# hermosayhl/CNN

Measured on AMD Instinct MI355X. Metric: images/sec (train step, 224x224x3), higher is better.
Workload: dtype f32; 1 GPU; reference AlexNet-style net (cpu/src/alexnet.cpp:10-33: 4x Conv3x3/s2 + ReLU, one MaxPool2x2, Linear 4608->3), full train step (fwd + softmax/CE + bwd + SGD), 224x224x3 fp32, BASELINE configs[1]; per_gpu_batch=256, global_batch=256, parallelism=dp1

## Files before the change

cnn_amd/csrc/common.h:

```cpp
#pragma once
#include <hip/hip_runtime.h>
#include <hip/hip_ext.h>

#include <atomic>
#include <cstdarg>
#include <cstdio>

#include "cnn_amd.h"

namespace cnn_amd {

char* error_buffer();
int fail(int code, const char* fmt, ...);

inline hipStream_t as_stream(void* s) { return reinterpret_cast<hipStream_t>(s); }

unsigned options_generation();
int num_cus();
struct DescMemo {
    struct Entry {
        cnn_conv2d_desc d;
        unsigned gen;
        int cus;
        bool used;
// ... 74 lines not shown
        if (e__ != hipSuccess)                                                                      \
            return ::cnn_amd::fail(CNN_AMD_E_HIP + (int)e__, "%s failed: %s", #expr, hipGetErrorString(e__)); \
    } while (0)

#define CNN_LAUNCH_CHECK() CNN_HIP_CHECK(hipGetLastError())

bool ktimer_active();
void ktimer_begin(hipStream_t s, const char* kernel, const char* fmt, ...);
void ktimer_end(hipStream_t s);

struct PublishState {
    hipEvent_t ev[2] = {nullptr, nullptr};
    int cur = 0, device = -1;
    bool armed = false;
    bool valid = false;
    bool stale = false;
    hipStream_t stream = nullptr;
};
PublishState& publish_state();
hipEvent_t publish_take(hipStream_t s);
int publish_after_launch(hipStream_t s);
void publish_mark_stale(hipStream_t s);
inline bool publish_busy() {
    const PublishState& p = publish_state();
    return p.armed || (p.valid && !p.stale);
}

template <typename... KArgs, typename... Args>
inline void launch_pub(void (*kern)(KArgs...), dim3 grid, dim3 block, unsigned shmem, hipStream_t s, Args&&... args) {
    hipEvent_t ev = publish_take(s);
    if (ev) hipExtLaunchKernelGGL(kern, grid, block, shmem, s, nullptr, ev, 0, static_cast<KArgs>(args)...);
    else hipLaunchKernelGGL(kern, grid, block, shmem, s, static_cast<KArgs>(args)...);
}

#define CNN_KLAUNCH(stream, kernel_name, expr, ...)                                         \
    do {                                                                                    \
        const bool t__ = ::cnn_amd::ktimer_active();                                        \
        if (t__) ::cnn_amd::ktimer_begin(stream, kernel_name, __VA_ARGS__);                 \
        expr;                                                                               \
        if (t__) ::cnn_amd::ktimer_end(stream);                                             \
        CNN_LAUNCH_CHECK();                                                                 \
        if (::cnn_amd::publish_busy())                                                      \
            if (int prc__ = ::cnn_amd::publish_after_launch(stream)) return prc__;          \
    } while (0)

#define CNN_REQUIRE(cond, ...)                                             \
    do {                                                                   \
        if (!(cond)) return ::cnn_amd::fail(CNN_AMD_E_BADARG, __VA_ARGS__); \
    } while (0)

__host__ __device__ inline int m16_filter_index(int j, int lane, int Ci, int slice) {
    return ((4 * (j / 9) + (lane >> 4)) * Ci + 16 * slice + (lane & 15)) * 9 + j % 9;
}

struct DeviceOnce {
    std::atomic<unsigned char> done[64];
    static int device() {
        int dev = 0;
        return (hipGetDevice(&dev) == hipSuccess && dev >= 0 && dev < 64) ? dev : -1;
    }
    bool needed() const {
        const int dev = device();
        return dev < 0 || done[dev].load(std::memory_order_acquire) == 0;
    }
    void mark() {
        const int dev = device();
        if (dev >= 0) done[dev].store(1, std::memory_order_release);
    }
};

__device__ __forceinline__ float sgd_one(float p, float g, float lr, float scale, bool scaled) {
#pragma clang fp contract(off)
    const float gs = scaled ? g * scale : g;
    const float step = lr * gs;
    return p - step;
}

template <bool kMomentum>
__device__ __forceinline__ float sgdm_one(float p, float g, float& v, float lr, float momentum, float wd, float scale, bool scaled,
                                          bool decay, bool nesterov) {
#pragma clang fp contract(off)
    const float gs = scaled ? g * scale : g;
    float d = gs;
    if (decay) {
        const float wp = wd * p;
        d = gs + wp;
    }
    float u = d;
    if (kMomentum) {
        const float mv = momentum * v;
        const float vn = mv + d;
        v = vn;
        if (nesterov) {
            const float mvn = momentum * vn;
            u = d + mvn;
        } else {
            u = vn;
        }
    }
    const float step = lr * u;
    return p - step;
}

constexpr int kWave = 64;
constexpr int kNumXCD = 8;

// ... 18 lines not shown
```

cnn_amd/csrc/conv_dgrad_rd.hip:

```cpp
#include <cstdlib>
#include <type_traits>

#include "common.h"

using namespace cnn_amd;

namespace cnn_amd {
bool igemm_preferred(const cnn_conv2d_desc* d, int mode);
}

namespace {

typedef float f32x16 __attribute__((ext_vector_type(16)));
struct __attribute__((packed, aligned(4))) f2u {
    float x, y;
};
struct __attribute__((packed, aligned(4))) f4u {
    float x, y, z, w;
};
typedef float v2f __attribute__((ext_vector_type(2)));
typedef float v4f __attribute__((ext_vector_type(4)));
struct Taps {
    v4f a, b;
    float c;
// ... 347 lines not shown
                const int g = g0 + ri, gp = g + NB - 1, rp = (ri + NB - 1) % NB;
                const bool wrap = gp >= G;
                const unsigned oo[3] = {wrap ? nxt.o[0] : cur.o[0], wrap ? nxt.o[1] : cur.o[1], wrap ? nxt.o[2] : cur.o[2]};
                load_group(ring[rp], wrap ? gp - G : gp, oo);
                RD_PIPE_FENCE(ring[ri].a[0][0][0]);
                (void)g;
#pragma unroll
                for (int u = 0; u < UC; ++u)
#pragma unroll
                    for (int kx = 0; kx < 3; ++kx) {
                        const f3u v = ring[ri].win[u][kx];
#pragma unroll
                        for (int ky = 0; ky < 3; ++ky) {
                            float d = cur.isz[ky] ? v.z : (cur.isy[ky] ? v.y : v.x);
                            d = cur.ok[kx][ky] ? d : 0.f;
#pragma unroll
                            for (int mt = 0; mt < MT; ++mt)
                                acc[mt] = __builtin_amdgcn_mfma_f32_32x32x2f32(ring[ri].a[u][mt][kx * 3 + ky], d, acc[mt], 0, 0, 0);
                        }
                    }
            }
        }
        if (cur.live) {
#pragma unroll
            for (int mt = 0; mt < MT; ++mt) {
                float m[16];
                if (p.relu_below) {
#pragma unroll
                    for (int r = 0; r < 16; ++r) {
                        const int rowl = mt * 32 + (r & 3) + 8 * (r >> 2) + 4 * kg;
                        m[r] = p.relu_below[(size_t)cur.xo + (size_t)(ci0 + rowl < p.Ci ? rowl : 0) * p.UV];
                    }
                }
#pragma unroll
                for (int r = 0; r < 16; ++r) {
                    const int rowl = mt * 32 + (r & 3) + 8 * (r >> 2) + 4 * kg;
                    if (ci0 + rowl >= p.Ci) continue;
                    float v = acc[mt][r];
                    if (p.relu_below) v = (m[r] <= 0.f) ? 0.f : v;
                    p.dx[(size_t)cur.xo + (size_t)rowl * p.UV] = v;
                }
            }
        }
        cur = nxt;
    }
}

#ifndef CNN_M16_DGRAD_NB
#define CNN_M16_DGRAD_NB 4
#endif
typedef float f32x4 __attribute__((ext_vector_type(4)));
constexpr unsigned kM16OOB = 0x7ffffffcu;

template <int CO, int NW, bool PREP, int KS, bool PD = false>
__global__ __launch_bounds__(NW * 64) void conv_dgrad_m16_s2_kernel(const DgRdParams p) {
    constexpr int C4 = CO / 4, NA = CO * 9 / 4;
    constexpr int NB = CNN_M16_DGRAD_NB;
    static_assert(C4 % NB == 0, "static ring indices");
    const int lane = threadIdx.x & 63;
    const int n = lane & 15, k = lane >> 4;
    const int slices = p.Ci >> 4;
    const int wid = xcd_swizzle(blockIdx.x, gridDim.x) * NW + (threadIdx.x >> 6);
    const int slice = wid % slices, half = KS > 1 ? (wid / slices) % KS : 0, wave_id = wid / (slices * KS);
    const int nwaves = p.tiles;
    const int groups = (p.pixels + 15) >> 4;
    if (wave_id >= nwaves || wave_id >= groups) return;
    float wa[NA];
    if constexpr (PREP) {
#pragma unroll
        for (int j = 0; j < NA; ++j) wa[j] = p.w[((half * slices + slice) * NA + j) * 64 + lane];
    } else {
#pragma unroll
        for (int j = 0; j < NA; ++j) wa[j] = p.w[half * CO * p.Ci * 9 + m16_filter_index(j, lane, p.Ci, slice)];
    }
    const int plane = p.Ho * p.Wo;
    const size_t hw = (size_t)p.H * p.W;
    const unsigned chs = (unsigned)hw * 4u;
    const bool odd = (p.W & 1) != 0;
    const __amdgpu_buffer_rsrc_t rsrc = __builtin_amdgcn_make_buffer_rsrc((void*)p.dy, 0, (int)((unsigned)p.B * CO * KS * plane * 4u), 0x00020000);
    const __amdgpu_buffer_rsrc_t xrs = __builtin_amdgcn_make_buffer_rsrc((void*)p.dx, 0, (int)((unsigned)p.B * p.Ci * (unsigned)hw * 4u), 0x00020000);
    const __amdgpu_buffer_rsrc_t mrs =
        __builtin_amdgcn_make_buffer_rsrc((void*)(p.relu_below ? p.relu_below : p.dx), 0, (int)((unsigned)p.B * p.Ci * (unsigned)hw * 4u), 0x00020000);
    struct Loc {
        unsigned o0, o1;
        bool ca, cb;
        unsigned x0, x1;
        bool w1;
        unsigned xq[2][2];
    };
    auto locate = [&](int g, Loc& L) {
        const int pix = g * 16 + n;
        const bool live = g < groups && pix < p.pixels;
        const int pp = live ? pix : 0;
        const int b = fdiv(pp, p.m_uv, p.UV);
        const int rem = pp - b * p.UV;
        const int u = fdiv(rem, p.m_v, p.V);
        const int v = rem - u * p.V;
        L.cb = v == 0;
        L.ca = !L.cb && v < p.Wo;
        const int cs = L.ca ? v - 1 : (L.cb ? 0 : p.Wo - 2);
        const unsigned base = (unsigned)((b * CO * KS + half * CO + k) * plane + u * p.Wo + cs) * 4u;
        L.o0 = (live && u < p.Ho) ? base : kM16OOB;
        L.o1 = (live && u >= 1) ? base - (unsigned)p.Wo * 4u : kM16OOB;
        if constexpr (PD) {
            const int y0 = 2 * u - 1, c0 = 2 * v - 1;
            const int xb = (int)((((size_t)b * p.Ci + 16 * slice + 4 * k) * hw) * 4u) + (y0 * p.W + c0) * 4;
#pragma unroll
            for (int ph = 0; ph < 2; ++ph)
#pragma unroll
                for (int pw = 0; pw < 2; ++pw) {
                    const bool ok = live && (unsigned)(y0 + ph) < (unsigned)p.H && (unsigned)(c0 + pw) < (unsigned)p.W;
                    L.xq[ph][pw] = ok ? (unsigned)(xb + (ph * p.W + pw) * 4) : kM16OOB;
                }
            L.x0 = L.x1 = kM16OOB;
            L.w1 = true;
        } else {
            const unsigned xb = (unsigned)(((size_t)b * p.Ci + 16 * slice + 4 * k) * hw + (size_t)(2 * u) * p.W + 2 * v) * 4u;
            L.x0 = live ? xb : kM16OOB;
            L.x1 = (live && 2 * u + 1 < p.H) ? xb + (unsigned)p.W * 4u : kM16OOB;
            L.w1 = 2 * v + 1 < p.W;
        }
    };
    auto load_g = [&](v2f (&buf)[2], int c4, const Loc& L) {
        const int so = c4 * 4 * plane * 4;
        buf[0] = __builtin_bit_cast(v2f, __builtin_amdgcn_raw_buffer_load_b64(rsrc, (int)L.o0, so, 0));
        buf[1] = __builtin_bit_cast(v2f, __builtin_amdgcn_raw_buffer_load_b64(rsrc, (int)L.o1, so, 0));
    };
    Loc cur, nxt;
    locate(wave_id, cur);
    v2f ring[NB][2];
#pragma unroll
    for (int i = 0; i < NB - 1; ++i) load_g(ring[i], i, cur);
    for (int g = wave_id; g < groups; g += nwaves) {
        locate(g + nwaves, nxt);
        v2f mk[4][2];
        if constexpr (PD) {
            if (p.relu_below && half == 0) {
#pragma unroll
                for (int r = 0; r < 4; ++r)
#pragma unroll
                    for (int ph = 0; ph < 2; ++ph) {
                        mk[r][ph].x = __builtin_bit_cast(float, __builtin_amdgcn_raw_buffer_load_b32(mrs, (int)cur.xq[ph][0], (int)(r * chs), 0));
                        mk[r][ph].y = __builtin_bit_cast(float, __builtin_amdgcn_raw_buffer_load_b32(mrs, (int)cur.xq[ph][1], (int)(r * chs), 0));
                    }
            }
        } else
        if (p.relu_below && half == 0) {
            const unsigned m0 = (cur.w1 || cur.x0 == kM16OOB) ? cur.x0 : cur.x0 - 4u, m1 = (cur.w1 || cur.x1 == kM16OOB) ? cur.x1 : cur.x1 - 4u;
#pragma unroll
            for (int r = 0; r < 4; ++r) {
                mk[r][0] = __builtin_bit_cast(v2f, __builtin_amdgcn_raw_buffer_load_b64(mrs, (int)m0, (int)(r * chs), 0));
                mk[r][1] = __builtin_bit_cast(v2f, __builtin_amdgcn_raw_buffer_load_b64(mrs, (int)m1, (int)(r * chs), 0));
            }
        }
        f32x4 acc[4];
#pragma unroll
        for (int c = 0; c < 4; ++c) acc[c] = f32x4{0.f, 0.f, 0.f, 0.f};
#pragma unroll
        for (int c4 = 0; c4 < C4; ++c4) {
            const int gn = c4 + NB - 1;
            load_g(ring[gn % NB], gn % C4, gn < C4 ? cur : nxt);
            RD_PIPE_FENCE(ring[c4 % NB][0]);
            const v2f r0 = ring[c4 % NB][0], r1 = ring[c4 % NB][1];
            const float d00 = cur.ca ? r0.y : (cur.cb ? r0.x : 0.f), d01 = cur.ca ? r0.x : (cur.cb ? 0.f : r0.y);
            const float d10 = cur.ca ? r1.y : (cur.cb ? r1.x : 0.f), d11 = cur.ca ? r1.x : (cur.cb ? 0.f : r1.y);
            const float* a = &wa[c4 * 9];
#define M16_STEP(ACC, A_, B_)                                              \
    ACC = __builtin_amdgcn_mfma_f32_16x16x4f32(A_, B_, ACC, 0, 0, 0); \
    __builtin_amdgcn_sched_barrier(0)
            M16_STEP(acc[1], a[1], d00);
            M16_STEP(acc[0], a[0], d00);
            M16_STEP(acc[2], a[3], d00);
            M16_STEP(acc[0], a[2], d01);
            M16_STEP(acc[3], a[4], d00);
            M16_STEP(acc[0], a[6], d10);
            M16_STEP(acc[1], a[7], d10);
            M16_STEP(acc[0], a[8], d11);
            M16_STEP(acc[2], a[5], d01);
#undef M16_STEP
        }
        if constexpr (KS > 1) {
            __shared__ float red[2][KS - 1][NW / KS][16][64];
            const int rb = ((g - wave_id) / nwaves) & 1;
            if (half > 0) {
#pragma unroll
                for (int c = 0; c < 4; ++c)
#pragma unroll
                    for (int r = 0; r < 4; ++r) red[rb][half - 1][slice][c * 4 + r][lane] = acc[c][r];
            }
            __syncthreads();
            if (half > 0) {
                cur = nxt;
                continue;
            }
#pragma unroll
            for (int h = 0; h < KS - 1; ++h)
#pragma unroll
                for (int c = 0; c < 4; ++c)
#pragma unroll
                    for (int r = 0; r < 4; ++r) acc[c][r] += red[rb][h][slice][c * 4 + r][lane];
        }
        if constexpr (PD) {
#pragma unroll
            for (int r = 0; r < 4; ++r)
#pragma unroll
                for (int ph = 0; ph < 2; ++ph) {
                    float v0 = acc[ph * 2][r], v1 = acc[ph * 2 + 1][r];
                    if (p.relu_below) {
                        v0 = (mk[r][ph].x <= 0.f) ? 0.f : v0;
                        v1 = (mk[r][ph].y <= 0.f) ? 0.f : v1;
                    }
                    __builtin_amdgcn_raw_buffer_store_b32(__builtin_bit_cast(unsigned, v0), xrs, (int)cur.xq[ph][0], (int)(r * chs), 0);
                    __builtin_amdgcn_raw_buffer_store_b32(__builtin_bit_cast(unsigned, v1), xrs, (int)cur.xq[ph][1], (int)(r * chs), 0);
                }
            cur = nxt;
            continue;
        }
        const unsigned pp0 = cur.w1 ? cur.x0 : kM16OOB, pp1 = cur.w1 ? cur.x1 : kM16OOB;
        const unsigned ss0 = cur.w1 ? kM16OOB : cur.x0, ss1 = cur.w1 ? kM16OOB : cur.x1;
#pragma unroll
        for (int r = 0; r < 4; ++r)
#pragma unroll
            for (int ph = 0; ph < 2; ++ph) {
                float v0 = acc[ph * 2][r], v1 = acc[ph * 2 + 1][r];
                if (p.relu_below) {
                    const float k0 = cur.w1 ? mk[r][ph].x : mk[r][ph].y;
                    v0 = (k0 <= 0.f) ? 0.f : v0;
                    v1 = (mk[r][ph].y <= 0.f) ? 0.f : v1;
                }
                typedef unsigned u2 __attribute__((ext_vector_type(2)));
                __builtin_amdgcn_raw_buffer_store_b64(__builtin_bit_cast(u2, v2f{v0, v1}), xrs, (int)(ph ? pp1 : pp0), (int)(r * chs), 0);
                if (odd) __builtin_amdgcn_raw_buffer_store_b32(__builtin_bit_cast(unsigned, v0), xrs, (int)(ph ? ss1 : ss0), (int)(r * chs), 0);
            }
        cur = nxt;
    }
}

inline unsigned magic_of(int d) { return (unsigned)((1ull << 32) / (unsigned)d) + 1u; }

struct DgRdPlan {
    DgRdParams p;
    int co, nw, cgroups, blocks_x, mt;
    bool m16;
    size_t lds, img_floats;
};

inline bool m16_wanted(const cnn_conv2d_desc* d) {
    if (d->s != 2 || !((d->Ci == 16 && d->Co == 32) || (d->Ci == 32 && d->Co == 64) || (d->Ci == 64 && d->Co == 128))) return false;
    if (d->pad != 0 && !(d->pad == 1 && d->Ci == 64 && d->Co == 128)) return false;
    if ((long long)d->B * d->Co * cnn_conv2d_out_dim(d->H, 3, 2, d->pad) * cnn_conv2d_out_dim(d->W, 3, 2, d->pad) >= (1ll << 29) ||
        (long long)d->B * d->Ci * d->H * d->W >= (1ll << 29))
        return false;
    const OptVal e = CNN_OPT_VAL("DGRAD_M16");
    if (e && atoi(e) == 0) return false;
    if (d->Ci >= 32 && e && atoi(e) == 1) return false;
    if (d->Ci == 64 && e && atoi(e) == 2) return false;
    return true;
}

bool make_plan(const cnn_conv2d_desc* d, DgRdPlan* pl) {
    if (d->k != 3 || (d->s != 2 && d->s != 1)) return false;
    if (d->pad != 0 && !(d->pad == 1 && d->s == 2 && m16_wanted(d))) return false;
    if (d->s == 1 && ((d->Co != 64 && d->Co != 128) || d->Ci % 32 != 0)) return false;
    if ((d->Co != 32 && d->Co != 64 && d->Co != 128) || d->Ci % 16 != 0) return false;
    pl->m16 = m16_wanted(d);
    if (d->Co == 32 && !pl->m16 && !((CNN_OPT_SET("DGRAD_RD32") && CNN_OPT_INT("DGRAD_RD32", 0) != 0))) return false;
    if (const OptVal e = CNN_OPT_VAL("DGRAD_RD"))
        if (atoi(e) == 0) return false;
    DgRdParams& p = pl->p;
    p.B = d->B; p.Ci = d->Ci; p.H = d->H; p.W = d->W;
    p.Ho = cnn_conv2d_out_dim(d->H, 3, d->s, d->pad);
    p.Wo = cnn_conv2d_out_dim(d->W, 3, d->s, d->pad);
    if (p.Ho < 1 || p.Wo < (d->s == 1 ? 3 : 2)) return false;
    if (d->s == 1) { p.U = d->H; p.V = d->W; }
    else { p.U = (d->H + 2 * d->pad + 1) / 2; p.V = (d->W + 2 * d->pad + 1) / 2; }
    p.UV = p.U * p.V;
    const long long pixels = (long long)d->B * p.UV;
    if (pixels >= (1ll << 30) || (long long)d->B * d->Ci * d->H * d->W >= (1ll << 31) || (long long)d->B * d->Co * p.Ho * p.Wo >= (1ll << 31))
        return false;
    p.pixels = (int)pixels;
    p.tiles = (int)((pixels + 31) / 32);
    p.m_uv = magic_of(p.UV);
    p.m_v = magic_of(p.V);
    p.dbg = CNN_MEASURE_INT("DGRAD_RD_DBG", 0);
    pl->co = d->Co;
    pl->mt = (d->s == 1 && d->Ci % 64 == 0) ? 2 : 1;
    if (const OptVal e = CNN_OPT_VAL("DGRAD_RD_MT")) pl->mt = (atoi(e) == 2 && d->s == 1 && d->Ci % 64 == 0) ? 2 : 1;
    pl->cgroups = (d->Ci + 32 * pl->mt - 1) / (32 * pl->mt);
// ... 18 lines not shown
    return true;
}

template <int CO, int NW>
int launch(const DgRdPlan& pl, hipStream_t s, const char* name, const cnn_conv2d_desc* d) {
    const int var = CNN_OPT_INT("DGRAD_RD_VAR", 0);
    auto kern = var == 3 ? conv_dgrad_rd_s2_kernel<CO, NW, 2, 2> : conv_dgrad_rd_s2_kernel<CO, NW, 2, 4>;
    const dim3 grid(pl.blocks_x, pl.cgroups);
    CNN_KLAUNCH(s, name, (kern<<<grid, NW * 64, pl.lds, s>>>(pl.p)), "B%d Ci%d %dx%d Co%d k%d s%d p%d", d->B, d->Ci, d->H, d->W,
                d->Co, d->k, d->s, d->pad);
    return CNN_AMD_OK;
}

inline int prepared_transposed() { return CNN_OPT_SET("DGRAD_RD_NOTR") ? 0 : 1; }

}

namespace cnn_amd {

bool dgrad_rd_supported(const cnn_conv2d_desc* d) {
    DgRdPlan pl;
    return make_plan(d, &pl);
}

size_t dgrad_rd_prepared_floats(const cnn_conv2d_desc* d) {
    DgRdPlan pl;
    return make_plan(d, &pl) ? pl.img_floats : 0;
}

int dgrad_rd_prepare_layout(const cnn_conv2d_desc* d, int* transposed) {
    DgRdPlan pl;
    if (!make_plan(d, &pl)) return 0;
    *transposed = pl.m16 ? 2 : prepared_transposed();
    return 1;
}

__global__ __launch_bounds__(256) void dgrad_rd_transpose_kernel(const float* __restrict__ w, float* __restrict__ img, int Co, int Ci) {
    const int total = Co * Ci * 9;
    for (int i = blockIdx.x * 256 + threadIdx.x; i < total; i += gridDim.x * 256) {
        const int ci = i % Ci, r = i / Ci, tap = r % 9, co = r / 9;
        img[i] = w[((size_t)co * Ci + ci) * 9 + tap];
    }
}

int dgrad_rd_backward_data(const cnn_conv2d_desc* d, const float* dy, const float* w, const float* img, const float* relu_below,
                           float* dx, void* ws, size_t ws_bytes, hipStream_t s) {
    DgRdPlan pl;
    if (!make_plan(d, &pl)) return fail(CNN_AMD_E_BADARG, "conv_dgrad_rd: geometry not covered");
    pl.p.dy = dy; pl.p.w = w ? w : img; pl.p.tr = w ? 0 : prepared_transposed(); pl.p.relu_below = relu_below; pl.p.dx = dx;
    if (pl.m16) {
        pl.p.tr = w ? 0 : 2;
        char nm[64];
        snprintf(nm, sizeof(nm), "conv_dgrad_rd<2,%d,m16>/dgrad%s", d->Co, relu_below ? "+relu" : "");
#define M16(CO_, PREP_, NW_, KS_)                                                                                                        \
    CNN_KLAUNCH(s, nm, (launch_pub(conv_dgrad_m16_s2_kernel<CO_, NW_, PREP_, KS_>, dim3(pl.blocks_x), dim3(NW_ * 64), 0, s, pl.p)), "B%d Ci%d %dx%d Co%d k%d s%d p%d", \
                d->B, d->Ci, d->H, d->W, d->Co, d->k, d->s, d->pad)
        if (d->Co == 32) { if (pl.p.tr == 2) M16(32, true, 4, 1); else M16(32, false, 4, 1); }
        else if (d->Co == 64) { if (pl.p.tr == 2) M16(64, true, 4, 1); else M16(64, false, 4, 1); }
        else if (d->pad == 1) {
#define M16P(PREP_)                                                                                                                        \
    CNN_KLAUNCH(s, nm, (launch_pub(conv_dgrad_m16_s2_kernel<64, 8, PREP_, 2, true>, dim3(pl.blocks_x), dim3(8 * 64), 0, s, pl.p)), "B%d Ci%d %dx%d Co%d k%d s%d p%d", \
                d->B, d->Ci, d->H, d->W, d->Co, d->k, d->s, d->pad)
            if (pl.p.tr == 2) M16P(true); else M16P(false);
#undef M16P
        }
        else { if (pl.p.tr == 2) M16(64, true, 8, 2); else M16(64, false, 8, 2); }
#undef M16
        return CNN_AMD_OK;
    }
    if (w && ws && ws_bytes >= pl.img_floats * sizeof(float) && prepared_transposed()) {
        const unsigned gx = (unsigned)((pl.img_floats + 255) / 256);
        CNN_KLAUNCH(s, "dgrad_rd_transpose", (dgrad_rd_transpose_kernel<<<gx > 512 ? 512 : gx, 256, 0, s>>>(w, (float*)ws, d->Co, d->Ci)),
                    "B%d Ci%d %dx%d Co%d k%d s%d p%d", d->B, d->Ci, d->H, d->W, d->Co, d->k, d->s, d->pad);
        pl.p.w = (const float*)ws;
        pl.p.tr = 1;
    }
    char name[64];
    snprintf(name, sizeof(name), "conv_dgrad_rd<2,%d>/dgrad%s", d->Co, relu_below ? "+relu" : "");
    if (d->s == 1) {
        const dim3 grid(pl.blocks_x, pl.cgroups);
        snprintf(name, sizeof(name), "conv_dgrad_rd<1,%d,%d>/dgrad%s", d->Co, pl.mt, relu_below ? "+relu" : "");
#define S1(CO_, MT_, UC_) CNN_KLAUNCH(s, name, (conv_dgrad_rd_s1_kernel<CO_, MT_, 4, UC_><<<grid, 256, 0, s>>>(pl.p)), "B%d Ci%d %dx%d Co%d k%d s%d p%d", \
                                      d->B, d->Ci, d->H, d->W, d->Co, d->k, d->s, d->pad)
        const int uc = CNN_OPT_INT("DGRAD_RD_UC", 1);
        if (d->Co == 64 && pl.mt == 2) S1(64, 2, 1);
        else if (d->Co == 64) { if (uc == 2) S1(64, 1, 2); else S1(64, 1, 1); }
        else if (pl.mt == 2) S1(128, 2, 1);
        else { if (uc == 2) S1(128, 1, 2); else S1(128, 1, 1); }
#undef S1
        return CNN_AMD_OK;
    }
    if (d->Ci == 16) {
        const dim3 grid(pl.blocks_x, pl.cgroups);
#define SH(CO_) CNN_KLAUNCH(s, name, (conv_dgrad_rd_s2_kernel<CO_, 4, 2, 4, true><<<grid, 256, 0, s>>>(pl.p)), "B%d Ci%d %dx%d Co%d k%d s%d p%d", \
                            d->B, d->Ci, d->H, d->W, d->Co, d->k, d->s, d->pad)
        if (d->Co == 32) SH(32); else if (d->Co == 64) SH(64); else SH(128);
#undef SH
        return CNN_AMD_OK;
    }
    if (d->Co == 32) return launch<32, 4>(pl, s, name, d);
    if (d->Co == 64) return launch<64, 4>(pl, s, name, d);
    return launch<128, 4>(pl, s, name, d);
}

}
```

cnn_amd/csrc/conv_fwd_rd.hip:

```cpp
#include <cstdlib>

#include "common.h"

using namespace cnn_amd;

namespace cnn_amd {
bool igemm_preferred(const cnn_conv2d_desc* d, int mode);
}

namespace {

typedef float f32x16 __attribute__((ext_vector_type(16)));
struct __attribute__((packed, aligned(4))) f3u {
    float x, y, z;
};

#define RD_PIPE_FENCE(reg) asm volatile("" : "+v"(reg) : : "memory")

struct FwdRdParams {
    const float* x;
    const float* w;
    const float* img;
    const float* bias;
    float* y;
// ... 116 lines not shown
    for (; tile < p.tiles; tile += tstep) {
        const bool more = tile + tstep < p.tiles;
        if (more) locate(tile + tstep, nxoff, nyoff, nlive);
        f32x16 acc[MT];
#pragma unroll
        for (int mt = 0; mt < MT; ++mt) acc[mt] = bias_r[mt];
#pragma unroll
        for (int g = 0; g < G; ++g) {
            const int bi = g & 1, ri = g % NB, gp = g + NB - 1;
            if (gp < G) load_group(xb[gp % NB], gp, xoff);
            else if (more) load_group(xb[gp % NB], gp - G, nxoff);
            load_filters(ab[bi ^ 1], g + 1 < G ? g + 1 : 0);
            RD_PIPE_FENCE(ab[bi][0]);
#pragma unroll
            for (int u = 0; u < UC; ++u)
#pragma unroll
                for (int kx = 0; kx < 3; ++kx) {
                    const f3u v = xb[ri][u * 3 + kx];
#pragma unroll
                    for (int ky = 0; ky < 3; ++ky) {
                        const float bv = ky == 0 ? v.x : ky == 1 ? v.y : v.z;
#pragma unroll
                        for (int mt = 0; mt < MT; ++mt)
                            acc[mt] = __builtin_amdgcn_mfma_f32_32x32x2f32(ab[bi][((u * 3 + kx) * 3 + ky) * MT + mt], bv, acc[mt], 0, 0, 0);
                    }
                }
        }
        const long long dbg_t2 = p.dbg ? clock64() : 0;
        if (live) {
#pragma unroll
            for (int mt = 0; mt < MT; ++mt)
#pragma unroll
                for (int r = 0; r < 16; ++r) {
                    const int rowl = mt * 32 + (r & 3) + 8 * (r >> 2);
                    if (co0 + rowl + 4 * kg < p.Co) {
                        const size_t o = (size_t)yoff + (size_t)rowl * p.HoWo;
                        const float v = acc[mt][r];
                        if (p.y) p.y[o] = v;
                        if (p.y2) p.y2[o] = v >= 0.f ? v : 0.f;
                    }
                }
        }
        if (p.dbg && threadIdx.x == 0 && (blockIdx.x | blockIdx.y) == 0)
            printf("conv_fwd_rd wg 0: upload %lld, to end of MFMAs %lld, stores issued %lld cycles after start\n", dbg_t1 - dbg_t0,
                   dbg_t2 - dbg_t0, clock64() - dbg_t0);
        xoff = nxoff;
        yoff = nyoff;
        live = nlive;
    }
}

typedef float f32x4 __attribute__((ext_vector_type(4)));

__host__ __device__ inline int m16f_filter_index(int i, int Ci) {
    const int NA = Ci * 9 / 4;
    const int lane = i & 63, j = (i >> 6) % NA, slice = (i >> 6) / NA;
    return ((16 * slice + (lane & 15)) * Ci + 4 * (j / 9) + (lane >> 4)) * 9 + j % 9;
}

template <int S, int CI, int NW, bool PREP, int NB, int MS>
__global__ __launch_bounds__(NW * 64) void conv_fwd_m16_kernel(const FwdRdParams p) {
    constexpr int C4 = CI / 4, NA = C4 * 9;
    static_assert(C4 % NB == 0, "static ring indices");
    const int lane = threadIdx.x & 63;
    const int n = lane & 15, k = lane >> 4;
    const int slices = (p.Co >> 4) / MS, parts = p.tiles;
    const int wid = xcd_swizzle(blockIdx.x, gridDim.x) * NW + (threadIdx.x >> 6);
    const int slice = wid % slices, part = wid / slices;
    const int groups = (p.pixels + 15) >> 4;
    if (part >= parts || part >= groups) return;
    float wa[MS][NA], bs[MS][4];
#pragma unroll
    for (int m = 0; m < MS; ++m) {
        const int sl = slice * MS + m;
        if constexpr (PREP) {
#pragma unroll
            for (int j = 0; j < NA; ++j) wa[m][j] = p.img[(sl * NA + j) * 64 + lane];
        } else {
#pragma unroll
            for (int j = 0; j < NA; ++j) wa[m][j] = p.w[((16 * sl + n) * CI + 4 * (j / 9) + k) * 9 + j % 9];
        }
#pragma unroll
        for (int r = 0; r < 4; ++r) bs[m][r] = p.bias[16 * sl + 4 * k + r];
    }
    const long long dbg_t0 = p.dbg ? clock64() : 0;
    long long dbg_t1 = 0;
    int dbg_groups = 0;
    const unsigned plane = (unsigned)(p.H * p.W);
    auto locate = [&](int g, unsigned& xoff, unsigned& yoff, bool& live) {
        const int pi = g * 16 + n;
        live = g < groups && pi < p.pixels;
        const int pic = live ? pi : p.pixels - 1;
        const int b = fdiv(pic, p.m_howo, p.HoWo), rem = pic - b * p.HoWo;
        const int pr = fdiv(rem, p.m_wo, p.Wo), q = rem - pr * p.Wo;
        xoff = (unsigned)((b * CI + k) * (int)plane + (S * pr) * p.W + S * q);
        yoff = (unsigned)((b * p.Co + 16 * MS * slice + 4 * k) * p.HoWo + rem);
    };
    auto load_g = [&](f3u (&buf)[3], int c4, unsigned xoff) {
#pragma unroll
        for (int kx = 0; kx < 3; ++kx) {
            const float* base = p.x + ((size_t)(c4 * 4) * plane + (size_t)kx * p.W);
            buf[kx] = *(const f3u*)(base + xoff);
        }
    };
    unsigned xoff, yoff, nxoff, nyoff;
    bool live, nlive;
    locate(part, xoff, yoff, live);
    f3u xb[NB][3];
#pragma unroll
    for (int i = 0; i < NB - 1; ++i) load_g(xb[i], i, xoff);
    for (int g = part; g < groups; g += parts) {
        locate(g + parts, nxoff, nyoff, nlive);
        constexpr int NACC = 2;
        f32x4 acc[MS][NACC];
#pragma unroll
        for (int m = 0; m < MS; ++m) {
            acc[m][0] = f32x4{bs[m][0], bs[m][1], bs[m][2], bs[m][3]};
#pragma unroll
            for (int a = 1; a < NACC; ++a) acc[m][a] = f32x4{0.f, 0.f, 0.f, 0.f};
        }
#pragma unroll
        for (int c4 = 0; c4 < C4; ++c4) {
            const int gn = c4 + NB - 1;
            load_g(xb[gn % NB], gn % C4, gn < C4 ? xoff : nxoff);
            RD_PIPE_FENCE(xb[c4 % NB][0].x);
#pragma unroll
            for (int i = 0; i < 9; ++i) {
                const f3u v = xb[c4 % NB][i / 3];
                const float bv = i % 3 == 0 ? v.x : i % 3 == 1 ? v.y : v.z;
                const int a = (c4 * 9 + i) % NACC;
#pragma unroll
                for (int m = 0; m < MS; ++m) {
                    acc[m][a] = __builtin_amdgcn_mfma_f32_16x16x4f32(wa[m][c4 * 9 + i], bv, acc[m][a], 0, 0, 0);
                    __builtin_amdgcn_sched_barrier(0);
                }
            }
        }
        if (live) {
#pragma unroll
            for (int mr = 0; mr < MS * 4; ++mr) {
                const int m = mr >> 2, r = mr & 3;
                const float v = acc[m][0][r] + acc[m][1][r];
                const size_t o = (size_t)yoff + (size_t)(16 * m + r) * p.HoWo;
                if (p.y) p.y[o] = v;
                if (p.y2) p.y2[o] = v >= 0.f ? v : 0.f;
            }
        }
        xoff = nxoff;
        yoff = nyoff;
        live = nlive;
        if (p.dbg) {
            if (!dbg_groups) dbg_t1 = clock64();
            ++dbg_groups;
        }
    }
    if (p.dbg && threadIdx.x == 0 && blockIdx.x == 0)
        printf("conv_fwd_m16 wg 0: first group done %lld, all %d groups %lld cycles after the filter loads were issued\n", dbg_t1 - dbg_t0, dbg_groups,
               clock64() - dbg_t0);
}

inline unsigned magic_of(int d) { return (unsigned)((1ull << 32) / (unsigned)d) + 1u; }

struct FwdRdPlan {
    FwdRdParams p;
    int s, ci, mt, nw, cgroups, blocks_x;
    bool m16;
    int m16_blocks, m16_parts, m16_ms;
    size_t lds, img_floats;
};

bool make_plan(const cnn_conv2d_desc* d, FwdRdPlan* pl) {
    if (d->k != 3 || d->pad != 0 || (d->s != 1 && d->s != 2)) return false;
    if (d->Ci != 16 && d->Ci != 32 && d->Ci != 64) return false;
    if (const OptVal e = CNN_OPT_VAL("FWD_RD"))
        if (atoi(e) == 0) return false;
    FwdRdParams& p = pl->p;
    p.B = d->B; p.H = d->H; p.W = d->W; p.Co = d->Co;
    p.Ho = cnn_conv2d_out_dim(d->H, 3, d->s, 0);
    p.Wo = cnn_conv2d_out_dim(d->W, 3, d->s, 0);
    if (p.Ho <= 0 || p.Wo <= 0) return false;
    p.HoWo = p.Ho * p.Wo;
    const long long pixels = (long long)d->B * p.HoWo;
    if (pixels >= (1ll << 30) || (long long)d->B * d->Ci * d->H * d->W >= (1ll << 31) || pixels * d->Co >= (1ll << 31)) return false;
    p.pixels = (int)pixels;
    p.tiles = (int)((pixels + 31) / 32);
    p.m_howo = magic_of(p.HoWo);
    p.m_wo = magic_of(p.Wo);
    p.dbg = CNN_MEASURE_INT("FWD_RD_DBG", 0);
    pl->s = d->s;
    pl->ci = d->Ci;
    const int mtiles = (d->Co + 31) / 32;
    int mt = mtiles >= 2 && (long long)p.tiles * ((mtiles + 1) / 2) >= 4 * 4 * num_cus() ? 2 : 1;
    if ((size_t)(mt * 32 + 1) * d->Ci * 9 * 4 > 96 * 1024) mt = 1;
    if (const OptVal e = CNN_OPT_VAL("FWD_RD_MT")) mt = atoi(e) == 2 && mtiles >= 2 ? 2 : 1;
    pl->mt = mt;
    pl->cgroups = (mtiles + mt - 1) / mt;
    pl->img_floats = ((size_t)(mt * 32 + 1) * d->Ci * 9 + mt * 32 + 3) / 4 * 4;
    pl->lds = pl->img_floats * sizeof(float);
    pl->nw = pl->lds > 80 * 1024 ? 8 : 4;
    const int env = CNN_OPT_INT("FWD_RD_BLOCKS", 0);
    long long bx = (env > 0 ? env : (pl->nw == 8 ? num_cus() : 2 * num_cus())) / pl->cgroups;
    const long long need = (p.tiles + pl->nw - 1) / pl->nw;
    if (bx > need) bx = need;
    if (bx < 1) bx = 1;
    pl->blocks_x = (int)bx;
    const bool m16_ok = d->Co % 16 == 0 && (long long)d->B * d->Ci * d->H * d->W < (1ll << 29);
    const bool thin = d->Ci == 16 && d->Co % 32 == 0 && !((CNN_OPT_SET("FWD_M16_THIN") && CNN_OPT_INT("FWD_M16_THIN", 0) == 0));
    pl->m16 = m16_ok && ((long long)p.tiles * mtiles < 4 * 4 * num_cus() || thin);
    if (const OptVal e = CNN_OPT_VAL("FWD_M16")) pl->m16 = m16_ok && atoi(e) != 0;
    if (pl->m16) {
        pl->m16_ms = (d->Co % 32 == 0 && d->Ci <= 32 && !((CNN_OPT_SET("FWD_M16_MS") && CNN_OPT_INT("FWD_M16_MS", 0) == 1))) ? 2 : 1;
        const int slices = d->Co / 16 / pl->m16_ms, groups = (int)((pixels + 15) / 16);
        int per_simd = CNN_OPT_INT("FWD_M16_WAVES", (d->Ci == 16 ? 2 : 1));
        if (per_simd < 1 || per_simd > 8) per_simd = 1;
        int parts = per_simd * 4 * num_cus() / slices;
        if (parts < 1) parts = 1;
        if (parts > groups) parts = groups;
        pl->m16_parts = parts;
        pl->m16_blocks = (parts * slices + 3) / 4;
    }
    if (!pl->m16 && cnn_amd::igemm_preferred(d, 0)) return false;
    return true;
}

template <int S, int CI, int MT, int NW>
int launch(const FwdRdPlan& pl, hipStream_t s, const char* name, const cnn_conv2d_desc* d) {
    auto kern = conv_fwd_rd_kernel<S, CI, MT, NW, 2>;
    static DeviceOnce attr_once;
    if (attr_once.needed()) {
        CNN_HIP_CHECK(hipFuncSetAttribute((const void*)kern, hipFuncAttributeMaxDynamicSharedMemorySize, 160 * 1024));
        attr_once.mark();
    }
    const dim3 grid(pl.blocks_x, pl.cgroups);
    CNN_KLAUNCH(s, name, (kern<<<grid, NW * 64, pl.lds, s>>>(pl.p)), "B%d Ci%d %dx%d Co%d k%d s%d p%d", d->B, d->Ci, d->H, d->W,
                d->Co, d->k, d->s, d->pad);
    return CNN_AMD_OK;
}

struct FwdRdPrepJob {
    int kind;
    const float* w;
    const float* bias;
    float* img;
    int Co, Ci, cb, img_floats, cgroups, tr;
};
struct FwdRdPrepBatch {
    FwdRdPrepJob job[12];
};

__global__ __launch_bounds__(256) void fwd_rd_prepare_kernel(const FwdRdPrepBatch pb) {
    const FwdRdPrepJob j = pb.job[blockIdx.y];
    if (j.kind == 2) {
        const int total = j.Co * j.Ci * 9;
        for (int i = blockIdx.x * 256 + threadIdx.x; i < total; i += gridDim.x * 256) j.img[i] = j.w[m16f_filter_index(i, j.Ci)];
        return;
    }
    if (j.kind == 1) {
        const int total = j.Co * j.Ci * 9;
        for (int i = blockIdx.x * 256 + threadIdx.x; i < total; i += gridDim.x * 256) {
            if (j.tr == 2) {
                const int coh = j.Co > 64 ? j.Co / 2 : j.Co, na = coh * 9 / 4, slices = j.Ci / 16;
                const int jj = (i >> 6) % na, blk = (i >> 6) / na, slice = blk % slices, half = blk / slices;
                j.img[i] = j.w[half * coh * j.Ci * 9 + m16_filter_index(jj, i & 63, j.Ci, slice)];
            } else if (j.tr) {
                const int ci = i % j.Ci, r = i / j.Ci, tap = r % 9, co = r / 9;
                j.img[i] = j.w[((size_t)co * j.Ci + ci) * 9 + tap];
            } else {
                j.img[i] = j.w[i];
            }
        }
        return;
    }
    const int K = j.Ci * 9, cbp = j.cb + 1, total = j.cgroups * j.img_floats;
    for (int i = blockIdx.x * 256 + threadIdx.x; i < total; i += gridDim.x * 256) {
        const int g = i / j.img_floats, o = i - g * j.img_floats;
        float v = 0.f;
        if (o < K * cbp) {
            const int k = o / cbp, c = o - k * cbp, co = g * j.cb + c;
            if (c < j.cb && co < j.Co) v = j.w[(size_t)co * K + k];
        } else if (o < K * cbp + j.cb) {
            const int co = g * j.cb + (o - K * cbp);
            if (co < j.Co) v = j.bias[co];
        }
        j.img[i] = v;
    }
}

}

namespace cnn_amd {

bool fwd_rd_supported(const cnn_conv2d_desc* d) {
    FwdRdPlan pl;
    return make_plan(d, &pl);
}
bool fwd_rd_small(const cnn_conv2d_desc* d) {
    FwdRdPlan pl;
    return make_plan(d, &pl) && pl.m16;
}

size_t fwd_rd_prepared_floats(const cnn_conv2d_desc* d) {
    FwdRdPlan pl;
    if (!make_plan(d, &pl)) return 0;
    const size_t a = pl.img_floats * pl.cgroups, b = (size_t)d->Co * d->Ci * 9;
    return a > b ? a : b;
}

int dgrad_rd_prepare_layout(const cnn_conv2d_desc* d, int* transposed);

int rd_prepare_batch(int n, const cnn_conv2d_desc* descs, const float* const* w, const float* const* bias, void* const* fwd,
                     void* const* dgrad, hipStream_t s, unsigned* fdone, unsigned* ddone) {
    FwdRdPrepBatch pb;
    int jobs = 0;
    size_t most = 0;
    for (int i = 0; i < n && i < 6; ++i) {
        FwdRdPlan pl;
        if (fwd && fwd[i] && !(*fdone >> i & 1u) && make_plan(&descs[i], &pl)) {
            CNN_REQUIRE(w[i] && bias[i], "cnn_conv2d_prepare_filters: filters / bias of layer %d are null", i);
            FwdRdPrepJob& j = pb.job[jobs++];
            j.kind = pl.m16 ? 2 : 0; j.w = w[i]; j.bias = bias[i]; j.img = (float*)fwd[i];
            j.Co = descs[i].Co; j.Ci = descs[i].Ci; j.cb = pl.mt * 32; j.img_floats = (int)pl.img_floats; j.cgroups = pl.cgroups; j.tr = 0;
            if (pl.img_floats * pl.cgroups > most) most = pl.img_floats * pl.cgroups;
            *fdone |= 1u << i;
        }
        int tr = 0;
        if (dgrad && dgrad[i] && !(*ddone >> i & 1u) && dgrad_rd_prepare_layout(&descs[i], &tr)) {
            CNN_REQUIRE(w[i] != nullptr, "cnn_conv2d_prepare_filters: filters of layer %d are null", i);
            FwdRdPrepJob& j = pb.job[jobs++];
            j.kind = 1; j.w = w[i]; j.bias = nullptr; j.img = (float*)dgrad[i];
            j.Co = descs[i].Co; j.Ci = descs[i].Ci; j.cb = 0; j.img_floats = 0; j.cgroups = 0; j.tr = tr;
            const size_t nf = (size_t)descs[i].Co * descs[i].Ci * 9;
            if (nf > most) most = nf;
            *ddone |= 1u << i;
        }
    }
    if (jobs) {
        unsigned gx = (unsigned)((most + 255) / 256);
        if (gx > 512) gx = 512;
        CNN_KLAUNCH(s, "rd_prepare", (fwd_rd_prepare_kernel<<<dim3(gx, jobs), 256, 0, s>>>(pb)), "jobs=%d", jobs);
    }
    return CNN_AMD_OK;
}

int fwd_rd_forward(const cnn_conv2d_desc* d, const float* x, const float* w, const float* img, const float* bias, float* y,
                   float* y_relu, hipStream_t s) {
    FwdRdPlan pl;
    if (!make_plan(d, &pl)) return fail(CNN_AMD_E_BADARG, "conv_fwd_rd: geometry not covered");
    pl.p.x = x; pl.p.w = w; pl.p.img = w ? nullptr : img; pl.p.bias = bias; pl.p.y = y; pl.p.y2 = y_relu;
    char name[64];
    if (pl.m16) {
        pl.p.tiles = pl.m16_parts;
        snprintf(name, sizeof(name), "conv_fwd_rd<%d,%d,m16>/fwd%s", d->s, d->Ci, y_relu ? "+relu" : "");
#define M16K(S_, CI_, PREP_, MS_)                                                                                                            \
    CNN_KLAUNCH(s, name, (launch_pub(conv_fwd_m16_kernel<S_, CI_, 4, PREP_, 4, MS_>, dim3(pl.m16_blocks), dim3(256), 0, s, pl.p)), "B%d Ci%d %dx%d Co%d k%d s%d p%d", \
                d->B, d->Ci, d->H, d->W, d->Co, d->k, d->s, d->pad)
#define M16(S_, CI_)                                                          \
    do {                                                                      \
        if (pl.m16_ms == 2 && CI_ <= 32) {                                    \
            if (pl.p.img) M16K(S_, (CI_ <= 32 ? CI_ : 32), true, 2);         \
            else M16K(S_, (CI_ <= 32 ? CI_ : 32), false, 2);                 \
        } else {                                                              \
            if (pl.p.img) M16K(S_, CI_, true, 1);                             \
            else M16K(S_, CI_, false, 1);                                     \
        }                                                                     \
    } while (0)
        if (d->s == 2) { if (d->Ci == 16) M16(2, 16); else if (d->Ci == 32) M16(2, 32); else M16(2, 64); }
        else { if (d->Ci == 16) M16(1, 16); else if (d->Ci == 32) M16(1, 32); else M16(1, 64); }
#undef M16K
#undef M16
        return CNN_AMD_OK;
    }
    snprintf(name, sizeof(name), "conv_fwd_rd<%d,%d,%d>/fwd%s", d->s, d->Ci, pl.mt, y_relu ? "+relu" : "");
#define GO(S_, CI_)                                                                                  \
    do {                                                                                             \
        if (pl.mt == 2 && pl.nw == 8) return launch<S_, CI_, 2, 8>(pl, s, name, d);                  \
        if (pl.mt == 2) return launch<S_, CI_, 2, 4>(pl, s, name, d);                                \
        if (pl.nw == 8) return launch<S_, CI_, 1, 8>(pl, s, name, d);                                \
        return launch<S_, CI_, 1, 4>(pl, s, name, d);                                                \
    } while (0)
    if (d->s == 2) {
        if (d->Ci == 16) GO(2, 16); else if (d->Ci == 32) GO(2, 32); else GO(2, 64);
    } else {
        if (d->Ci == 16) GO(1, 16); else if (d->Ci == 32) GO(1, 32); else GO(1, 64);
    }
#undef GO
    return CNN_AMD_OK;
}

}
```

Measured before the change: 606,700 images/sec.

## Stream m16 conv filter loads into first group and vectorize prepacked filter image

The m16 forward and dgrad conv kernels used to load all filter registers before starting the input pipeline. Now they load only the first ring slices up front and fetch the rest per channel chunk inside the first group's loop, so filter fetch overlaps the input and gradient loads. The prepared filter image is re-laid out so each lane reads a 16-byte float4 quad, with a scalar fallback when the image is not 16-byte aligned. The rework adds template variants and a debug timing path, and may raise register pressure or change the instruction schedule.

```diff
diff --git a/cnn_amd/csrc/common.h b/cnn_amd/csrc/common.h
--- a/cnn_amd/csrc/common.h
+++ b/cnn_amd/csrc/common.h
@@ -150,6 +150,30 @@
 __host__ __device__ inline int m16_filter_index(int j, int lane, int Ci, int slice) {
     return ((4 * (j / 9) + (lane >> 4)) * Ci + 16 * slice + (lane & 15)) * 9 + j % 9;
 }
+__host__ __device__ inline int m16f_filter_index(int j, int lane, int Ci, int slice) {
+    return ((16 * slice + (lane & 15)) * Ci + 4 * (j / 9) + (lane >> 4)) * 9 + j % 9;
+}
+
+struct M16Slot {
+    int bank, j, lane;
+};
+__host__ __device__ inline M16Slot m16_image_slot(int i, int NA) {
+    const int q = i >> 2, na4 = NA / 4;
+    return M16Slot{(q >> 6) / na4, 4 * ((q >> 6) % na4) + (i & 3), q & 63};
+}
+#define M16_INLINE __attribute__((always_inline))
+#define M16_MEM_FENCE() asm volatile("" ::: "memory")
+template <bool V16>
+__device__ __forceinline__ void m16_load_quad(const float* img, int bank, int na4, int j4, int lane, float* r) {
+    const float* q = img + (size_t)__builtin_amdgcn_readfirstlane((bank * na4 + j4) * 256);
+    if constexpr (V16) {
+        const float4 v = ((const float4*)q)[lane];
+        r[0] = v.x; r[1] = v.y; r[2] = v.z; r[3] = v.w;
+    } else {
+#pragma unroll
+        for (int e = 0; e < 4; ++e) r[e] = q[4 * lane + e];
+    }
+}
 
 struct DeviceOnce {
     std::atomic<unsigned char> done[64];
diff --git a/cnn_amd/csrc/conv_dgrad_rd.hip b/cnn_amd/csrc/conv_dgrad_rd.hip
--- a/cnn_amd/csrc/conv_dgrad_rd.hip
+++ b/cnn_amd/csrc/conv_dgrad_rd.hip
@@ -423,9 +423,10 @@
 typedef float f32x4 __attribute__((ext_vector_type(4)));
 constexpr unsigned kM16OOB = 0x7ffffffcu;
 
-template <int CO, int NW, bool PREP, int KS, bool PD = false>
+template <int CO, int NW, int FL, int KS, bool PD = false>
 __global__ __launch_bounds__(NW * 64) void conv_dgrad_m16_s2_kernel(const DgRdParams p) {
     constexpr int C4 = CO / 4, NA = CO * 9 / 4;
+    static_assert(NA % 4 == 0, "whole 16-byte elements");
     constexpr int NB = CNN_M16_DGRAD_NB;
     static_assert(C4 % NB == 0, "static ring indices");
     const int lane = threadIdx.x & 63;
@@ -436,14 +437,6 @@
     const int nwaves = p.tiles;
     const int groups = (p.pixels + 15) >> 4;
     if (wave_id >= nwaves || wave_id >= groups) return;
-    float wa[NA];
-    if constexpr (PREP) {
-#pragma unroll
-        for (int j = 0; j < NA; ++j) wa[j] = p.w[((half * slices + slice) * NA + j) * 64 + lane];
-    } else {
-#pragma unroll
-        for (int j = 0; j < NA; ++j) wa[j] = p.w[half * CO * p.Ci * 9 + m16_filter_index(j, lane, p.Ci, slice)];
-    }
     const int plane = p.Ho * p.Wo;
     const size_t hw = (size_t)p.H * p.W;
     const unsigned chs = (unsigned)hw * 4u;
@@ -492,7 +485,7 @@
             L.w1 = 2 * v + 1 < p.W;
         }
     };
-    auto load_g = [&](v2f (&buf)[2], int c4, const Loc& L) {
+    auto load_g = [&](v2f (&buf)[2], int c4, const Loc& L) M16_INLINE {
         const int so = c4 * 4 * plane * 4;
         buf[0] = __builtin_bit_cast(v2f, __builtin_amdgcn_raw_buffer_load_b64(rsrc, (int)L.o0, so, 0));
         buf[1] = __builtin_bit_cast(v2f, __builtin_amdgcn_raw_buffer_load_b64(rsrc, (int)L.o1, so, 0));
@@ -502,9 +495,8 @@
     v2f ring[NB][2];
 #pragma unroll
     for (int i = 0; i < NB - 1; ++i) load_g(ring[i], i, cur);
-    for (int g = wave_id; g < groups; g += nwaves) {
-        locate(g + nwaves, nxt);
-        v2f mk[4][2];
+    v2f mk[4][2];
+    auto load_mask = [&]() M16_INLINE {
         if constexpr (PD) {
             if (p.relu_below && half == 0) {
 #pragma unroll
@@ -524,6 +516,29 @@
                 mk[r][1] = __builtin_bit_cast(v2f, __builtin_amdgcn_raw_buffer_load_b64(mrs, (int)m1, (int)(r * chs), 0));
             }
         }
+    };
+    load_mask();
+    M16_MEM_FENCE();
+    float wa[NA];
+    auto load_filters = [&](int c0, int c1) M16_INLINE {
+        if constexpr (FL != 0) {
+#pragma unroll
+            for (int j4 = 0; j4 < NA / 4; ++j4)
+                if (4 * j4 >= 9 * c0 && 4 * j4 < 9 * c1) m16_load_quad<FL == 2>(p.w, half * slices + slice, NA / 4, j4, lane, &wa[4 * j4]);
+        } else {
+#pragma unroll
+            for (int j = 0; j < NA; ++j)
+                if (j >= 9 * c0 && j < 9 * c1) wa[j] = p.w[half * CO * p.Ci * 9 + m16_filter_index(j, lane, p.Ci, slice)];
+        }
+    };
+    load_filters(0, NB - 1);
+    M16_MEM_FENCE();
+    const long long dbg_t0 = p.dbg ? clock64() : 0;
+    long long dbg_t1 = 0;
+    int dbg_groups = 0;
+    auto group = [&](int g, bool first) M16_INLINE {
+        locate(g + nwaves, nxt);
+        if (!first) load_mask();
         f32x4 acc[4];
 #pragma unroll
         for (int c = 0; c < 4; ++c) acc[c] = f32x4{0.f, 0.f, 0.f, 0.f};
@@ -531,6 +546,7 @@
         for (int c4 = 0; c4 < C4; ++c4) {
             const int gn = c4 + NB - 1;
             load_g(ring[gn % NB], gn % C4, gn < C4 ? cur : nxt);
+            if (first && gn < C4) load_filters(gn, gn + 1);
             RD_PIPE_FENCE(ring[c4 % NB][0]);
             const v2f r0 = ring[c4 % NB][0], r1 = ring[c4 % NB][1];
             const float d00 = cur.ca ? r0.y : (cur.cb ? r0.x : 0.f), d01 = cur.ca ? r0.x : (cur.cb ? 0.f : r0.y);
@@ -562,7 +578,7 @@
             __syncthreads();
             if (half > 0) {
                 cur = nxt;
-                continue;
+                return;
             }
 #pragma unroll
             for (int h = 0; h < KS - 1; ++h)
@@ -585,7 +601,11 @@
                     __builtin_amdgcn_raw_buffer_store_b32(__builtin_bit_cast(unsigned, v1), xrs, (int)cur.xq[ph][1], (int)(r * chs), 0);
                 }
             cur = nxt;
-            continue;
+            if (p.dbg) {
+                if (!dbg_groups) dbg_t1 = clock64();
+                ++dbg_groups;
+            }
+            return;
         }
         const unsigned pp0 = cur.w1 ? cur.x0 : kM16OOB, pp1 = cur.w1 ? cur.x1 : kM16OOB;
         const unsigned ss0 = cur.w1 ? kM16OOB : cur.x0, ss1 = cur.w1 ? kM16OOB : cur.x1;
@@ -604,7 +624,16 @@
                 if (odd) __builtin_amdgcn_raw_buffer_store_b32(__builtin_bit_cast(unsigned, v0), xrs, (int)(ph ? ss1 : ss0), (int)(r * chs), 0);
             }
         cur = nxt;
-    }
+        if (p.dbg) {
+            if (!dbg_groups) dbg_t1 = clock64();
+            ++dbg_groups;
+        }
+    };
+    group(wave_id, true);
+    for (int g = wave_id + nwaves; g < groups; g += nwaves) group(g, false);
+    if (p.dbg && threadIdx.x == 0 && blockIdx.x == 0)
+        printf("conv_dgrad_m16 wg 0: first group done %lld, all %d groups %lld cycles after the filter loads were issued\n", dbg_t1 - dbg_t0,
+               dbg_groups, clock64() - dbg_t0);
 }
 
 inline unsigned magic_of(int d) { return (unsigned)((1ull << 32) / (unsigned)d) + 1u; }
@@ -729,19 +758,20 @@
         pl.p.tr = w ? 0 : 2;
         char nm[64];
         snprintf(nm, sizeof(nm), "conv_dgrad_rd<2,%d,m16>/dgrad%s", d->Co, relu_below ? "+relu" : "");
-#define M16(CO_, PREP_, NW_, KS_)                                                                                                        \
-    CNN_KLAUNCH(s, nm, (launch_pub(conv_dgrad_m16_s2_kernel<CO_, NW_, PREP_, KS_>, dim3(pl.blocks_x), dim3(NW_ * 64), 0, s, pl.p)), "B%d Ci%d %dx%d Co%d k%d s%d p%d", \
+#define M16(CO_, FL_, NW_, KS_)                                                                                                          \
+    CNN_KLAUNCH(s, nm, (launch_pub(conv_dgrad_m16_s2_kernel<CO_, NW_, FL_, KS_>, dim3(pl.blocks_x), dim3(NW_ * 64), 0, s, pl.p)), "B%d Ci%d %dx%d Co%d k%d s%d p%d", \
                 d->B, d->Ci, d->H, d->W, d->Co, d->k, d->s, d->pad)
-        if (d->Co == 32) { if (pl.p.tr == 2) M16(32, true, 4, 1); else M16(32, false, 4, 1); }
-        else if (d->Co == 64) { if (pl.p.tr == 2) M16(64, true, 4, 1); else M16(64, false, 4, 1); }
+        const int fl = w ? 0 : ((uintptr_t)img % 16 == 0 ? 2 : 1);
+        if (d->Co == 32) { if (fl == 2) M16(32, 2, 4, 1); else if (fl == 1) M16(32, 1, 4, 1); else M16(32, 0, 4, 1); }
+        else if (d->Co == 64) { if (fl == 2) M16(64, 2, 4, 1); else if (fl == 1) M16(64, 1, 4, 1); else M16(64, 0, 4, 1); }
         else if (d->pad == 1) {
-#define M16P(PREP_)                                                                                                                        \
-    CNN_KLAUNCH(s, nm, (launch_pub(conv_dgrad_m16_s2_kernel<64, 8, PREP_, 2, true>, dim3(pl.blocks_x), dim3(8 * 64), 0, s, pl.p)), "B%d Ci%d %dx%d Co%d k%d s%d p%d", \
+#define M16P(FL_)                                                                                                                          \
+    CNN_KLAUNCH(s, nm, (launch_pub(conv_dgrad_m16_s2_kernel<64, 8, FL_, 2, true>, dim3(pl.blocks_x), dim3(8 * 64), 0, s, pl.p)), "B%d Ci%d %dx%d Co%d k%d s%d p%d", \
                 d->B, d->Ci, d->H, d->W, d->Co, d->k, d->s, d->pad)
-            if (pl.p.tr == 2) M16P(true); else M16P(false);
+            if (fl == 2) M16P(2); else if (fl == 1) M16P(1); else M16P(0);
 #undef M16P
         }
-        else { if (pl.p.tr == 2) M16(64, true, 8, 2); else M16(64, false, 8, 2); }
+        else { if (fl == 2) M16(64, 2, 8, 2); else if (fl == 1) M16(64, 1, 8, 2); else M16(64, 0, 8, 2); }
 #undef M16
         return CNN_AMD_OK;
     }
diff --git a/cnn_amd/csrc/conv_fwd_rd.hip b/cnn_amd/csrc/conv_fwd_rd.hip
--- a/cnn_amd/csrc/conv_fwd_rd.hip
+++ b/cnn_amd/csrc/conv_fwd_rd.hip
@@ -192,16 +192,11 @@
 
 typedef float f32x4 __attribute__((ext_vector_type(4)));
 
-__host__ __device__ inline int m16f_filter_index(int i, int Ci) {
-    const int NA = Ci * 9 / 4;
-    const int lane = i & 63, j = (i >> 6) % NA, slice = (i >> 6) / NA;
-    return ((16 * slice + (lane & 15)) * Ci + 4 * (j / 9) + (lane >> 4)) * 9 + j % 9;
-}
-
-template <int S, int CI, int NW, bool PREP, int NB, int MS>
+template <int S, int CI, int NW, int FL, int NB, int MS>
 __global__ __launch_bounds__(NW * 64) void conv_fwd_m16_kernel(const FwdRdParams p) {
     constexpr int C4 = CI / 4, NA = C4 * 9;
     static_assert(C4 % NB == 0, "static ring indices");
+    static_assert(NA % 4 == 0, "whole 16-byte elements");
     const int lane = threadIdx.x & 63;
     const int n = lane & 15, k = lane >> 4;
     const int slices = (p.Co >> 4) / MS, parts = p.tiles;
@@ -209,23 +204,6 @@
     const int slice = wid % slices, part = wid / slices;
     const int groups = (p.pixels + 15) >> 4;
     if (part >= parts || part >= groups) return;
-    float wa[MS][NA], bs[MS][4];
-#pragma unroll
-    for (int m = 0; m < MS; ++m) {
-        const int sl = slice * MS + m;
-        if constexpr (PREP) {
-#pragma unroll
-            for (int j = 0; j < NA; ++j) wa[m][j] = p.img[(sl * NA + j) * 64 + lane];
-        } else {
-#pragma unroll
-            for (int j = 0; j < NA; ++j) wa[m][j] = p.w[((16 * sl + n) * CI + 4 * (j / 9) + k) * 9 + j % 9];
-        }
-#pragma unroll
-        for (int r = 0; r < 4; ++r) bs[m][r] = p.bias[16 * sl + 4 * k + r];
-    }
-    const long long dbg_t0 = p.dbg ? clock64() : 0;
-    long long dbg_t1 = 0;
-    int dbg_groups = 0;
     const unsigned plane = (unsigned)(p.H * p.W);
     auto locate = [&](int g, unsigned& xoff, unsigned& yoff, bool& live) {
         const int pi = g * 16 + n;
@@ -236,7 +214,7 @@
         xoff = (unsigned)((b * CI + k) * (int)plane + (S * pr) * p.W + S * q);
         yoff = (unsigned)((b * p.Co + 16 * MS * slice + 4 * k) * p.HoWo + rem);
     };
-    auto load_g = [&](f3u (&buf)[3], int c4, unsigned xoff) {
+    auto load_g = [&](f3u (&buf)[3], int c4, unsigned xoff) M16_INLINE {
 #pragma unroll
         for (int kx = 0; kx < 3; ++kx) {
             const float* base = p.x + ((size_t)(c4 * 4) * plane + (size_t)kx * p.W);
@@ -246,10 +224,38 @@
     unsigned xoff, yoff, nxoff, nyoff;
     bool live, nlive;
     locate(part, xoff, yoff, live);
+    float wa[MS][NA], bs[MS][4];
+#pragma unroll
+    for (int m = 0; m < MS; ++m)
+#pragma unroll
+        for (int r = 0; r < 4; ++r) bs[m][r] = p.bias[16 * (slice * MS + m) + 4 * k + r];
     f3u xb[NB][3];
 #pragma unroll
     for (int i = 0; i < NB - 1; ++i) load_g(xb[i], i, xoff);
-    for (int g = part; g < groups; g += parts) {
+    M16_MEM_FENCE();
+    auto load_filters = [&](int c0, int c1) M16_INLINE {
+        if constexpr (FL != 0) {
+#pragma unroll
+            for (int j4 = 0; j4 < NA / 4; ++j4)
+                if (4 * j4 >= 9 * c0 && 4 * j4 < 9 * c1) {
+#pragma unroll
+                    for (int m = 0; m < MS; ++m) m16_load_quad<FL == 2>(p.img, slice * MS + m, NA / 4, j4, lane, &wa[m][4 * j4]);
+                }
+        } else {
+#pragma unroll
+            for (int j = 0; j < NA; ++j)
+                if (j >= 9 * c0 && j < 9 * c1) {
+#pragma unroll
+                    for (int m = 0; m < MS; ++m) wa[m][j] = p.w[m16f_filter_index(j, lane, CI, slice * MS + m)];
+                }
+        }
+    };
+    load_filters(0, NB - 1);
+    M16_MEM_FENCE();
+    const long long dbg_t0 = p.dbg ? clock64() : 0;
+    long long dbg_t1 = 0;
+    int dbg_groups = 0;
+    auto group = [&](int g, bool first) M16_INLINE {
         locate(g + parts, nxoff, nyoff, nlive);
         constexpr int NACC = 2;
         f32x4 acc[MS][NACC];
@@ -263,6 +269,7 @@
         for (int c4 = 0; c4 < C4; ++c4) {
             const int gn = c4 + NB - 1;
             load_g(xb[gn % NB], gn % C4, gn < C4 ? xoff : nxoff);
+            if (first && gn < C4) load_filters(gn, gn + 1);
             RD_PIPE_FENCE(xb[c4 % NB][0].x);
 #pragma unroll
             for (int i = 0; i < 9; ++i) {
@@ -293,7 +300,9 @@
             if (!dbg_groups) dbg_t1 = clock64();
             ++dbg_groups;
         }
-    }
+    };
+    group(part, true);
+    for (int g = part + parts; g < groups; g += parts) group(g, false);
     if (p.dbg && threadIdx.x == 0 && blockIdx.x == 0)
         printf("conv_fwd_m16 wg 0: first group done %lld, all %d groups %lld cycles after the filter loads were issued\n", dbg_t1 - dbg_t0, dbg_groups,
                clock64() - dbg_t0);
@@ -392,16 +401,20 @@
     const FwdRdPrepJob j = pb.job[blockIdx.y];
     if (j.kind == 2) {
         const int total = j.Co * j.Ci * 9;
-        for (int i = blockIdx.x * 256 + threadIdx.x; i < total; i += gridDim.x * 256) j.img[i] = j.w[m16f_filter_index(i, j.Ci)];
+        for (int i = blockIdx.x * 256 + threadIdx.x; i < total; i += gridDim.x * 256) {
+            const M16Slot t = m16_image_slot(i, j.Ci * 9 / 4);
+            j.img[i] = j.w[m16f_filter_index(t.j, t.lane, j.Ci, t.bank)];
+        }
         return;
     }
     if (j.kind == 1) {
         const int total = j.Co * j.Ci * 9;
         for (int i = blockIdx.x * 256 + threadIdx.x; i < total; i += gridDim.x * 256) {
             if (j.tr == 2) {
-                const int coh = j.Co > 64 ? j.Co / 2 : j.Co, na = coh * 9 / 4, slices = j.Ci / 16;
-                const int jj = (i >> 6) % na, blk = (i >> 6) / na, slice = blk % slices, half = blk / slices;
-                j.img[i] = j.w[half * coh * j.Ci * 9 + m16_filter_index(jj, i & 63, j.Ci, slice)];
+                const int coh = j.Co > 64 ? j.Co / 2 : j.Co, slices = j.Ci / 16;
+                const M16Slot t = m16_image_slot(i, coh * 9 / 4);
+                const int slice = t.bank % slices, half = t.bank / slices;
+                j.img[i] = j.w[half * coh * j.Ci * 9 + m16_filter_index(t.j, t.lane, j.Ci, slice)];
             } else if (j.tr) {
                 const int ci = i % j.Ci, r = i / j.Ci, tap = r % 9, co = r / 9;
                 j.img[i] = j.w[((size_t)co * j.Ci + ci) * 9 + tap];
@@ -491,17 +504,20 @@
     if (pl.m16) {
         pl.p.tiles = pl.m16_parts;
         snprintf(name, sizeof(name), "conv_fwd_rd<%d,%d,m16>/fwd%s", d->s, d->Ci, y_relu ? "+relu" : "");
-#define M16K(S_, CI_, PREP_, MS_)                                                                                                            \
-    CNN_KLAUNCH(s, name, (launch_pub(conv_fwd_m16_kernel<S_, CI_, 4, PREP_, 4, MS_>, dim3(pl.m16_blocks), dim3(256), 0, s, pl.p)), "B%d Ci%d %dx%d Co%d k%d s%d p%d", \
+        const int fl = !pl.p.img ? 0 : ((uintptr_t)pl.p.img % 16 == 0 ? 2 : 1);
+#define M16K(S_, CI_, FL_, MS_)                                                                                                              \
+    CNN_KLAUNCH(s, name, (launch_pub(conv_fwd_m16_kernel<S_, CI_, 4, FL_, 4, MS_>, dim3(pl.m16_blocks), dim3(256), 0, s, pl.p)), "B%d Ci%d %dx%d Co%d k%d s%d p%d", \
                 d->B, d->Ci, d->H, d->W, d->Co, d->k, d->s, d->pad)
 #define M16(S_, CI_)                                                          \
     do {                                                                      \
         if (pl.m16_ms == 2 && CI_ <= 32) {                                    \
-            if (pl.p.img) M16K(S_, (CI_ <= 32 ? CI_ : 32), true, 2);         \
-            else M16K(S_, (CI_ <= 32 ? CI_ : 32), false, 2);                 \
+            if (fl == 2) M16K(S_, (CI_ <= 32 ? CI_ : 32), 2, 2);              \
+            else if (fl == 1) M16K(S_, (CI_ <= 32 ? CI_ : 32), 1, 2);         \
+            else M16K(S_, (CI_ <= 32 ? CI_ : 32), 0, 2);                      \
         } else {                                                              \
-            if (pl.p.img) M16K(S_, CI_, true, 1);                             \
-            else M16K(S_, CI_, false, 1);                                     \
+            if (fl == 2) M16K(S_, CI_, 2, 1);                                 \
+            else if (fl == 1) M16K(S_, CI_, 1, 1);                            \
+            else M16K(S_, CI_, 0, 1);                                         \
         }                                                                     \
     } while (0)
         if (d->s == 2) { if (d->Ci == 16) M16(2, 16); else if (d->Ci == 32) M16(2, 32); else M16(2, 64); }
```

Result: faster. 617,500 images/sec (median of 6 runs) (+1.8%).
